# wujinzhong/seamlessCloneOptimization

Hardware: AMD Instinct MI355X
Metric: Mpix/s seamlessClone (ROI 2048^2) (higher is better)
Workload: dtype f32 (arithmetic); storage: 16-bit fixed-point field on the first two level-0 stores of a solve, float16 right-hand side and level 1

## Files before the change

include/seamlessclone_hip_testing.h:

```cpp
#ifndef SEAMLESSCLONE_HIP_TESTING_H
#define SEAMLESSCLONE_HIP_TESTING_H

#include "seamlessclone_hip.h"

#ifdef __cplusplus
extern "C" {
#endif

#define SC_FLAG_LEGACY_PATHS   (1 << 6)
#define SC_LEGACY_SEPARATE_RESTRICT 1
#define SC_LEGACY_BOTTOM_F32   2
#define SC_LEGACY_SEPARATE_TAIL 4
#define SC_LEGACY_UNPACKED_TILES 8
#define SC_FLAG_KEEP_FIELD     (1 << 7)

#define SC_FLAG_POISON_ARENA   (1 << 14)


SC_API int sc_hip_mask_stage(void *instance, const uint8_t *mask, int mask_cols, int mask_rows, int mask_step,
                      int centerX, int centerY, int geo[6], uint8_t *M_out, size_t M_capacity);

SC_API int sc_hip_build_rhs(void *instance,
                     const uint8_t *face, int face_cols, int face_rows, int face_step,
                     const uint8_t *body, int body_cols, int body_rows, int body_step,
                     const uint8_t *mask, int mask_cols, int mask_rows, int mask_step,
                     int centerX, int centerY, int geo[6], float *B_out, float *lap_out, size_t plane_capacity);

SC_API int sc_hip_edit_rhs(void *instance, const sc_edit_params *p, const uint8_t *src, int cols, int rows, int src_step,
// ... 12 lines not shown
SC_API int sc_hip_field_finish(void *instance, uint8_t *body, int body_cols, int body_rows, int body_step, int ltx, int lty);
SC_API int sc_hip_field_lowmode(void *instance);

SC_API int sc_hip_field_time_sweeps(void *instance, int method, int launches, int sweeps_per_launch, float omega,
                             float *ms_per_launch);

SC_API int sc_hip_time_cycle0(void *instance, int launches, float *ms_per_launch);
SC_API int sc_hip_time_cycle0_form(void *instance, int form, int launches, float *ms_per_launch);
SC_API int sc_hip_time_coarse_chain(void *instance, int reps, float *ms_eager, float *ms_graph, int *launches);
SC_API int sc_hip_time_tail_phases(void *instance, unsigned long long *cycles11);

SC_API int sc_hip_selftest_host(void);

SC_API int sc_hip_cycle0_form(const int *facts, int index, int form[3]);

SC_API int sc_hip_coarse_tile_plan(const int *facts, int *plan);

#define SC_FUSED_ROW 18
SC_API int sc_hip_fused_schedule(const int *facts, const int *verdicts, int nverdicts, int *rows, int capacity);

SC_API int sc_hip_restore_spans(long long step, int rows, int ltx, int lty, int W, int H, long long *spans, int capacity);

#ifdef __cplusplus
}
#endif
#endif
```

seamlesscloneoptimization_amd/capi.py:

```python
from __future__ import annotations

import ctypes as C
import os
import re
import subprocess

import numpy as np

_PKG = os.path.dirname(os.path.abspath(__file__))
_ROOT = os.path.dirname(_PKG)
LIB_PATH = os.path.join(_PKG, "libseamlessclone_hip.so")
HEADER_PATH = os.path.join(_ROOT, "include", "seamlessclone_hip.h")
TESTING_HEADER_PATH = os.path.join(_ROOT, "include", "seamlessclone_hip_testing.h")

SC_OK = 0
SC_ERR_BAD_ARG = -1
SC_ERR_BAD_SIZE = -2
SC_ERR_EMPTY_MASK = -3
SC_ERR_ROI_OOB = -4
SC_ERR_HIP = -5
SC_ERR_NOT_CONVERGED = -6

SC_NORMAL_CLONE = 1
SC_MIXED_CLONE = 2
# ... 14 lines not shown
SC_METHOD_FFT = 6
SC_AUTO_DIRECT_MAX = 720
SC_AUTO_DIRECT_AREA = 450000
SC_AUTO_NARROW_MAX = 140
SC_AUTO_THIN_MAX = 4
SC_AUTO_THIN_LONG_MAX = 4096

SC_FLAG_NO_SPECULATE = 1 << 0
SC_FLAG_FLOAT_RHS = 1 << 1
SC_FLAG_FLOAT_U0 = 1 << 2
SC_FLAG_NO_COMPOSE_L1 = 1 << 3
SC_FLAG_VCYCLE_BOTTOM = 1 << 4
SC_FLAG_EXACT_TABLES = 1 << 5
SC_FLAG_LEGACY_PATHS = 1 << 6
SC_LEGACY_SEPARATE_RESTRICT, SC_LEGACY_BOTTOM_F32, SC_LEGACY_SEPARATE_TAIL, SC_LEGACY_UNPACKED_TILES = 1, 2, 4, 8
SC_FLAG_KEEP_FIELD = 1 << 7
SC_FLAG_FFT_FP64 = 1 << 8
SC_FLAG_OPENCV_GREY_MASK = 1 << 9
SC_FLAG_FLOAT_L1 = 1 << 10
SC_FLAG_FLOAT_FIELD = 1 << 11
SC_FLAG_NO_STAGE_MARKS = 1 << 12
SC_FLAG_ROWS_RETURN = 1 << 13
SC_FLAG_POISON_ARENA = 1 << 14

def auto_takes_direct(w: int, h: int) -> bool:
    if w <= SC_AUTO_DIRECT_MAX and h <= SC_AUTO_DIRECT_MAX:
        return True
    if max(w, h) <= SC_AUTO_THIN_LONG_MAX and (w * h <= SC_AUTO_DIRECT_AREA or min(w, h) <= SC_AUTO_NARROW_MAX):
        return True
    return False
# ... 234 lines not shown
    L.sc_hip_device_count.restype = C.c_int
    L.sc_hip_device_pci_bus_id.argtypes = [C.c_int, C.c_char_p, C.c_int]
    L.sc_hip_device_pci_bus_id.restype = C.c_int
    L.sc_hip_mask_stage.argtypes = [C.c_void_p] + _IMG + [C.c_int, C.c_int, i32p, u8p, C.c_size_t]
    L.sc_hip_mask_stage.restype = C.c_int
    L.sc_hip_build_rhs.argtypes = [C.c_void_p] + _IMG * 3 + [C.c_int, C.c_int, i32p, f32p, f32p, C.c_size_t]
    L.sc_hip_build_rhs.restype = C.c_int
    L.sc_hip_field_load.argtypes = [C.c_void_p, C.c_int, C.c_int, C.c_int, f32p, f32p]
    L.sc_hip_field_load.restype = C.c_int
    L.sc_hip_field_sweep.argtypes = [C.c_void_p, C.c_int, C.c_int, C.c_float, C.c_int]
    L.sc_hip_field_sweep.restype = C.c_int
    L.sc_hip_field_residual.argtypes = [C.c_void_p, f64p]
    L.sc_hip_field_residual.restype = C.c_int
    L.sc_hip_field_solve.argtypes = [C.c_void_p]
    L.sc_hip_field_solve.restype = C.c_int
    L.sc_hip_field_shape.argtypes = [C.c_void_p, i32p]
    L.sc_hip_field_shape.restype = C.c_int
    L.sc_hip_field_store.argtypes = [C.c_void_p, f32p, C.c_size_t]
    L.sc_hip_field_store.restype = C.c_int
    L.sc_hip_field_finish.argtypes = [C.c_void_p, C.c_void_p, C.c_int, C.c_int, C.c_int, C.c_int, C.c_int]
    L.sc_hip_field_finish.restype = C.c_int
    L.sc_hip_field_lowmode.argtypes = [C.c_void_p]
    L.sc_hip_field_lowmode.restype = C.c_int
    L.sc_hip_field_time_sweeps.argtypes = [C.c_void_p, C.c_int, C.c_int, C.c_int, C.c_float, C.POINTER(C.c_float)]
    L.sc_hip_field_time_sweeps.restype = C.c_int
    L.sc_hip_pool_create.argtypes = [C.c_int, C.c_int]
    L.sc_hip_pool_create.restype = C.c_void_p
    L.sc_hip_pool_destroy.argtypes = [C.c_void_p]
    L.sc_hip_pool_destroy.restype = None
    L.sc_hip_pool_size.argtypes = [C.c_void_p]
# ... 588 lines not shown
        cap = m[1] * m[2]
        B = np.zeros(3 * cap, np.float32)
        lap = np.zeros(3 * cap, np.float32)
        self._check(self.L.sc_hip_build_rhs(self.h, *f, *b, *m, int(cx), int(cy), geo.ctypes.data_as(i32p),
                                            B.ctypes.data_as(f32p), lap.ctypes.data_as(f32p), cap))
        W, H = int(geo[2]), int(geo[3])
        return geo, B[:3 * W * H].reshape(3, H, W).copy(), lap[:3 * W * H].reshape(3, H, W).copy()

    def field_load(self, U, lap):
        U = np.ascontiguousarray(U, np.float32)
        lap = np.ascontiguousarray(lap, np.float32)
        assert U.shape == lap.shape and U.ndim == 3
        Cc, H, W = U.shape
        self._check(self.L.sc_hip_field_load(self.h, W, H, Cc, U.ctypes.data_as(f32p), lap.ctypes.data_as(f32p)))

    def field_shape(self):
        whc = np.zeros(3, np.int32)
        self._check(self.L.sc_hip_field_shape(self.h, whc.ctypes.data_as(i32p)))
        return int(whc[2]), int(whc[1]), int(whc[0])

    def field_sweep(self, method, sweeps, omega=1.0, sweeps_per_launch=1):
        self._check(self.L.sc_hip_field_sweep(self.h, int(method), int(sweeps), float(omega), int(sweeps_per_launch)))

    def field_residual(self):
        out = np.zeros(2, np.float64)
        self._check(self.L.sc_hip_field_residual(self.h, out.ctypes.data_as(f64p)))
        return float(out[0]), float(out[1])

    def field_solve(self, allow_not_converged=False):
        rc = self.L.sc_hip_field_solve(self.h)
# ... 167 lines not shown

def plan_prepare(sizes, opts: "SolverOpts | None" = None) -> int:
    wh = np.ascontiguousarray(np.asarray(sizes, np.int32).reshape(-1, 2))
    return int(load().sc_hip_plan_prepare(wh.ctypes.data_as(i32p), wh.shape[0], C.byref(opts) if opts is not None else None))


def plan_cache_clear() -> None:
    load().sc_hip_plan_cache_clear()


CYCLE0_FACTS = ("sweeps", "prolong", "f_half", "u_half", "q16_in", "q16_out", "final_cycle", "out_bytes", "composed", "l1_half", "timing",
                "bands", "rag")


def cycle0_form(**facts):
    f = (C.c_int * len(CYCLE0_FACTS))(*[int(facts.pop(k, 0)) for k in CYCLE0_FACTS])
    if facts:
        raise TypeError("cycle0_form: no such fact: %s" % sorted(facts))
    out = (C.c_int * 3)()
    return tuple(out) if load().sc_hip_cycle0_form(f, 0, out) == 0 else -1


def coarse_tile_plan(W, H, C_, useful, halo, rows, size_class=False, unpacked=False, lanes=False):
    f = (C.c_int * 10)(W, H, C_, useful, halo, rows, int(size_class), int(unpacked), 0, 0)
    head = np.zeros(4, np.int32)
    rc = load().sc_hip_coarse_tile_plan(f, head.ctypes.data_as(i32p))
    if rc != 0:
        raise SeamlessCloneError(rc, "coarse_tile_plan")
    if not lanes:
        return tuple(int(v) for v in head)
# ... 80 lines not shown
```

seamlesscloneoptimization_amd/csrc/sc_common.h:

```cpp
#pragma once
#include <hip/hip_runtime.h>
#include <stdint.h>
#include <stddef.h>
#include <algorithm>
#include <string>
#include <vector>
#include "../../include/seamlessclone_hip_testing.h"

namespace sc {

struct Field {
    float *p = nullptr;
    int W = 0, H = 0, C = 0;
    int pitch = 0;
    size_t plane = 0;
    __host__ __device__ float *at(int c) const { return p + (size_t)c * plane; }
    size_t bytes() const { return plane * (size_t)C * sizeof(float); }
};

static inline int round_up(int v, int m) { return (v + m - 1) / m * m; }

struct Geo { int x0, y0, W, H, ltx, lty; };

struct Img8 {
// ... 198 lines not shown
struct MGGeom { MGDim x, y; };
struct ComposeArgs { Field E2; MGGeom g1; };

constexpr int C0_TIMING   = 1;
constexpr int C0_F_HALF   = 2;
constexpr int C0_U_HALF   = 4;
constexpr int C0_FINAL    = 8;
constexpr int C0_COMPOSED = 16;
constexpr int C0_OUT      = 32;
constexpr int C0_BANDS    = 64;
constexpr int C0_L1_HALF  = 128;
constexpr int C0_Q16_IN   = 256;
constexpr int C0_Q16_OUT  = 512;
constexpr int C0_PACK_ROWS = 6;
constexpr int C0_PACK     = 2048;
constexpr int C0_RAG      = 1024;

struct Cycle0Launch {
    Field Uin, Uout, F, Fc, E;
    MGGeom g{};
    int sweeps = 0;
    bool prolong = false;
    bool f_half = false, u_half = false, q16_in = false, q16_out = false;
    bool final_cycle = false, out_bytes = false;
    bool composed = false;
    bool l1_half = false, timing = false;
    ComposeArgs comp{};
    float4 *bands = nullptr;
    float *partial = nullptr;
    LmNodes lm{};
    AbortFlag sat{};
    const RagMember *rag = nullptr;
    hipStream_t s = nullptr;
};
bool cycle0_form(const Cycle0Launch &d, int &T, bool &PRO, int &TAG);
int  cycle0_form_at(int i, int &T, bool &PRO, int &TAG);
int  launch_cycle0(const Cycle0Launch &d);

constexpr int RAG_MAX_LEVELS = 12;
// ... 44 lines not shown
```

seamlesscloneoptimization_amd/csrc/sc_cycle0.hip:

```cpp
#include "sc_common.h"
#include <hip/hip_fp16.h>
#include "sc_wave.h"
#include "sc_mg_device.h"
#include <type_traits>

namespace sc {

constexpr int C0_HXQ = 3;
constexpr int C0_HX = 4 * C0_HXQ;

template <int R>
__device__ __forceinline__ void c0_load(const float *__restrict__ p, int P, int H, int x, int y0, float4 (&v)[R])
{
    const int xc = min(max(x, 0), P - 4);
#pragma unroll
    for (int r = 0; r < R; ++r) {
        const int yc = min(max(y0 + r, 0), H - 1);
        v[r] = *reinterpret_cast<const float4 *>(p + (size_t)yc * P + xc);
    }
}

template <int R>
__device__ __forceinline__ void c0_load_half(const __half *__restrict__ p, int P, int H, int x, int y0, float4 (&v)[R])
{
// ... 64 lines not shown
    else asm("v_fma_mix_f32 %0, %1, %2, %3 op_sel_hi:[0,0,1]" : "=v"(d) : "v"(s), "s"(quarter), "v"(raw));
    return d;
}
template <int K>
__device__ __forceinline__ float c0_f_minus(const uint2 &h, float s)
{
    const unsigned raw = (K < 2) ? h.x : h.y;
    float d;
    if (K & 1) asm("v_fma_mix_f32 %0, %1, -4.0, -%2 op_sel:[1,0,0] op_sel_hi:[1,0,0]" : "=v"(d) : "v"(raw), "v"(s));
    else asm("v_fma_mix_f32 %0, %1, -4.0, -%2 op_sel_hi:[1,0,0]" : "=v"(d) : "v"(raw), "v"(s));
    return d;
}
__device__ __forceinline__ float c0_comp(const float4 &v, int k) { return k == 0 ? v.x : k == 1 ? v.y : k == 2 ? v.z : v.w; }


template <int T, int NW, int R, bool PRO, bool GEN, bool ZEROIN, int TAG = 0>
__global__ __launch_bounds__(NW * 64) __attribute__((amdgpu_waves_per_eu(4))) void k_cycle0(Field Uin, Field Uout, Field F, Field Fc, Field E, MGGeom g,
                                                    float *__restrict__ partial, ComposeArgs comp, float4 *__restrict__ bands, LmNodes lm, AbortFlag sat,
                                                    const RagMember *__restrict__ rag, int lev)
{
    constexpr int HY = 2 * T + 2, RH = NW * R;
    constexpr bool RAG = (TAG & C0_RAG) != 0;
    constexpr bool COMP = (TAG & C0_COMPOSED) != 0;
    static_assert(!COMP || (PRO && !GEN && R % 2 == 0), "composition of two prolongations exists on level 0 only");
    constexpr bool FINAL = (TAG & C0_FINAL) != 0;
    constexpr bool OUT = (TAG & C0_OUT) != 0, BANDS = ((TAG & C0_BANDS) != 0 || FINAL) && !OUT;
    static_assert(!OUT || (FINAL && !GEN), "bytes leave from the last level-0 launch only");
    static_assert(!(TAG & C0_BANDS) || !GEN, "cell shares exist on level 0 only");
    constexpr bool HF = (TAG & C0_F_HALF) != 0, HU = (TAG & C0_U_HALF) != 0;
    static_assert(!(HF && GEN), "float16 right-hand sides exist on level 0 only");
    constexpr bool L1H = (TAG & C0_L1_HALF) != 0;
    constexpr bool UQI = (TAG & C0_Q16_IN) != 0, UQO = (TAG & C0_Q16_OUT) != 0;
    static_assert(!((UQI || UQO) && (GEN || (HU && UQI) || (OUT && UQO))), "16-bit fields: level 0, between its launches");
    static_assert(!L1H || !GEN || ZEROIN, "float16 level-1 fields: the level-1 launch starts from a zero correction");
    static_assert(!(PRO && GEN), "the in-kernel prolongation relies on level 0's regular last interval");
    static_assert(2 * T + 2 <= C0_HX, "column halo too small");
    static_assert(R % 2 == 0, "bands must hold whole coarse-row pairs");
    __shared__ float4 edge[2][NW][2][64];
    __shared__ float2 hedge[2][NW][64];
    const int lane = threadIdx.x & 63;
    const int wv = __builtin_amdgcn_readfirstlane(threadIdx.x >> 6);
    int W = Uin.W, H = Uin.H;
    const int P = Uin.pitch;
    const int nbx = (W + (256 - 2 * C0_HX) - 1) / (256 - 2 * C0_HX), nby = (H + (RH - 2 * HY) - 1) / (RH - 2 * HY);
    const int tile = xcd_tile(blockIdx.x, gridDim.x);
    constexpr bool PACK = (TAG & C0_PACK) != 0;
    static_assert(!PACK || (GEN && ZEROIN && !PRO && !RAG), "packed column tiles: the coarse forms of one size");
    TileLane tl{};
    if constexpr (PACK) tl = coarse_tile_lane(coarse_tile_plan(W, H, Uin.C, 256 - 2 * C0_HX, C0_HX, RH - 2 * HY, false), Uin.C, 256 - 2 * C0_HX, C0_HX, tile, lane);
    const int bx = tile % nbx, by = PACK ? tl.by : (tile / nbx) % nby;
    const int c = PACK ? min(tl.c, Uin.C - 1) : tile / (nbx * nby);
    const int sl = PACK ? tl.sl : lane, lps = PACK ? tl.lps : 64;
    const bool live = !PACK || tl.c < Uin.C;
    if constexpr (RAG) {
        const RagMember &m = rag[c / 3];
        W = m.lw[lev]; H = m.lh[lev];
        if (bx * (256 - 2 * C0_HX) >= W || by * (RH - 2 * HY) >= H) {
            if (PRO && threadIdx.x == 0) partial[tile] = 0.f;
            return;
        }
        g = m.g[lev];
        if (PRO) E.H = m.lh[lev + 1];
        if ((TAG & C0_COMPOSED) != 0) { comp.g1 = m.g[lev + 1]; comp.E2.H = m.lh[lev + 2]; }
    }
    const int x = PACK ? tl.x : bx * (256 - 2 * C0_HX) - C0_HX + 4 * lane;
    const int y0 = by * (RH - 2 * HY) - HY + wv * R;
    float4 u[R], f[HF ? 1 : R];
    uint2 fh[HF ? R : 1];
    if (ZEROIN) {
#pragma unroll
        for (int r = 0; r < R; ++r) u[r] = make_float4(0.f, 0.f, 0.f, 0.f);
    } else if (HU) {
        c0_load_half<R>(reinterpret_cast<const __half *>(Uin.p) + (size_t)c * Uin.plane, P, H, x, y0, u);
    } else if (UQI) {
        c0_load_q16<R>(reinterpret_cast<const uint16_t *>(Uin.p) + (size_t)c * Uin.plane, P, H, x, y0, u);
    } else {
        c0_load<R>(Uin.at(c), P, H, x, y0, u);
    }
    constexpr int NE = R / 2 + 2, NQ = R / 4 + 3;
    float2 eab[PRO ? NE : 1];
    float ecc[PRO ? NE : 1];
// ... 135 lines not shown
                    m2 = fmaxf(fmaxf(m2, fabsf(Sj.y)), fabsf(Sj.w));
                }
                Sp = Sj;
            }
            m = fmaxf(m1, fmaxf(0.5f * m2, 0.25f * m4));
        };
        if (inner) prolong(std::false_type{});
        else if (x >= 0 && x <= W - 2 && y0 + R - 1 >= 1 && y0 <= H - 2) prolong(std::true_type{});
        if constexpr (HF) c0_load_half_raw<R>(reinterpret_cast<const __half *>(F.p) + (size_t)c * F.plane, P, H, x, y0, fh);
        else c0_load<R>(F.at(c), P, H, x, y0, f);
#pragma unroll
        for (int o = 32; o > 0; o >>= 1) m = fmaxf(m, __shfl_xor(m, o, 64));
        __shared__ float red[NW];
        if (lane == 0) red[wv] = m;
        __syncthreads();
        if (threadIdx.x == 0) {
            float mm = red[0];
#pragma unroll
            for (int w = 1; w < NW; ++w) mm = fmaxf(mm, red[w]);
            partial[tile] = mm;
        }
    }

    if constexpr (!GEN) {
#pragma unroll
        for (int r = 0; r < R; ++r) {
            if constexpr (HF) c0_scale_q(fh[r]);
            else f[r] = make_float4(-0.25f * f[r].x, -0.25f * f[r].y, -0.25f * f[r].z, -0.25f * f[r].w);
        }
    }
    const float quarter = 0.25f;
    (void)quarter;
    float cw0 = (GEN && x + 0 == g.x.n) ? g.x.cw_last : 1.0f, dx0 = (GEN && x + 0 == g.x.n) ? g.x.d_last : 2.0f;
    float cw1 = (GEN && x + 1 == g.x.n) ? g.x.cw_last : 1.0f, dx1 = (GEN && x + 1 == g.x.n) ? g.x.d_last : 2.0f;
    float cw2 = (GEN && x + 2 == g.x.n) ? g.x.cw_last : 1.0f, dx2 = (GEN && x + 2 == g.x.n) ? g.x.d_last : 2.0f;
// ... 167 lines not shown
                v1 = __builtin_fmaf(h1[r + 1], 0.5f, __builtin_fmaf(m1, 0.5f, h1[r]));
            }
            const float fy = (J == g.y.nc) ? 2.0f * g.y.inv_last : 1.0f;
            if constexpr (L1H && !GEN) {
                __half *o = reinterpret_cast<__half *>(Fc.p) + (size_t)c * Fc.plane + (size_t)J * Fc.pitch + I;
                if (I >= 1 && I <= g.x.nc) o[0] = __float2half_rn(v0 * (fx0 * fy));
                if (I + 1 >= 1 && I + 1 <= g.x.nc) o[1] = __float2half_rn(v1 * (fx1 * fy));
            } else {
            float *o = fc + (size_t)J * Fc.pitch + I;
            if (I >= 1 && I <= g.x.nc) o[0] = v0 * (fx0 * fy);
            if (I + 1 >= 1 && I + 1 <= g.x.nc) o[1] = v1 * (fx1 * fy);
            }
        }
    }

    if (sl < C0_HXQ || sl >= lps - C0_HXQ || !live || x >= P || x >= W) return;
    if constexpr (OUT) {
        uint8_t *__restrict__ q = reinterpret_cast<uint8_t *>(Uout.p) + (size_t)c * Uout.plane;
        const bool corr = lm.CN && x <= W - 2;
        const int Yc0 = max(y0, 0) >> 3;
        float nd[3][2] = { { 0.f, 0.f }, { 0.f, 0.f }, { 0.f, 0.f } };
        if (corr) {
            const float *__restrict__ pn = lm.CN + (size_t)c * lm.ny * lm.npitch + (x >> 3);
#pragma unroll
            for (int k = 0; k < 3; ++k) {
                const float *row = pn + (size_t)min(Yc0 + k, lm.ny - 1) * lm.npitch;
                nd[k][0] = row[0]; nd[k][1] = row[1];
            }
        }
#pragma unroll
        for (int r = 0; r < R; ++r) {
            const int yr = wv * R + r, y = y0 + r;
            if (!(yr >= HY && yr < RH - HY && y >= 1 && y <= H - 2)) continue;
            float4 v = u[r];
            if (corr) {
                const bool second = (y >> 3) != Yc0;
                lm_add4_nodes(second ? nd[1][0] : nd[0][0], second ? nd[1][1] : nd[0][1], second ? nd[2][0] : nd[1][0], second ? nd[2][1] : nd[1][1], x, y, v);
            }
            *reinterpret_cast<unsigned *>(q + (size_t)y * P + x) = lm_byte(v.x) | (lm_byte(v.y) << 8) | (lm_byte(v.z) << 16) | (lm_byte(v.w) << 24);
        }
        return;
    }
    if constexpr (GEN && L1H) {
        __half *__restrict__ outh = reinterpret_cast<__half *>(Uout.p) + (size_t)c * Uout.plane;
#pragma unroll
        for (int r = 0; r < R; ++r) {
            const int yr = wv * R + r, y = y0 + r;
            if (!(yr >= HY && yr < RH - HY && y >= 0 && y < H)) continue;
            const __half2 a = __floats2half2_rn(u[r].x, u[r].y), b2 = __floats2half2_rn(u[r].z, u[r].w);
            uint2 pk; pk.x = *reinterpret_cast<const unsigned *>(&a); pk.y = *reinterpret_cast<const unsigned *>(&b2);
            *reinterpret_cast<uint2 *>(outh + (size_t)y * P + x) = pk;
        }
        return;
    }
    if constexpr (UQO) {
        uint16_t *__restrict__ outq = reinterpret_cast<uint16_t *>(Uout.p) + (size_t)c * Uout.plane;
// ... 4 lines not shown
            if (!(yr >= HY && yr < RH - HY && y >= 0 && y < H)) continue;
            uint2 pk;
            pk.x = c0_q16_checked(u[r].x, s0) | (c0_q16_checked(u[r].y, s1) << 16);
            pk.y = c0_q16_checked(u[r].z, s2) | (c0_q16_checked(u[r].w, s3) << 16);
            *reinterpret_cast<uint2 *>(outq + (size_t)y * P + x) = pk;
        }
        const int seen = s0 | (x + 1 < W ? s1 : 0) | (x + 2 < W ? s2 : 0) | (x + 3 < W ? s3 : 0);
        if ((seen & ~0xffff) && sat.p) { *sat.p = sat.gen; if (sat.host) *sat.host = sat.gen; }
        return;
    }
    float *__restrict__ out = Uout.at(c);
#pragma unroll
    for (int r = 0; r < R; ++r) {
        const int yr = wv * R + r, y = y0 + r;
        if (yr >= HY && yr < RH - HY && y >= 0 && y < H) *reinterpret_cast<float4 *>(out + (size_t)y * P + x) = u[r];
    }
}

constexpr int C0_NW = 8, C0_R = 8;


using Cycle0Kernel = void (*)(Field, Field, Field, Field, Field, MGGeom, float *, ComposeArgs, float4 *, LmNodes, AbortFlag, const RagMember *, int);
struct Cycle0Form { int T; bool PRO; int TAG; Cycle0Kernel k; };
#define C0_FORM(T_, PRO_, TAG_) { T_, PRO_, TAG_, k_cycle0<T_, C0_NW, C0_R, PRO_, false, false, TAG_> }
#define C0_FORM_RAG(T_, PRO_, TAG_) C0_FORM(T_, PRO_, TAG_), C0_FORM(T_, PRO_, TAG_ | C0_RAG)
#define C0_FORM_TWIN(T_, PRO_, TAG_) C0_FORM(T_, PRO_, TAG_), C0_FORM(T_, PRO_, TAG_ | C0_TIMING)
constexpr int C0_FAST = C0_F_HALF | C0_L1_HALF, C0_FAST_CYCLE = C0_FAST | C0_COMPOSED, C0_Q16 = C0_Q16_IN | C0_Q16_OUT;
static constexpr Cycle0Form c0_forms[] = {
    C0_FORM_RAG(2, false, C0_FAST | C0_U_HALF | C0_Q16_OUT), C0_FORM(2, false, C0_FAST | C0_U_HALF | C0_Q16_OUT | C0_TIMING),
    C0_FORM_RAG(2, false, C0_FAST | C0_U_HALF), C0_FORM_RAG(2, false, C0_FAST),
// ... 6 lines not shown
    C0_FORM_TWIN(4, true, C0_COMPOSED | C0_F_HALF), C0_FORM(4, true, C0_COMPOSED | C0_F_HALF | C0_BANDS),
    C0_FORM(2, true, C0_COMPOSED | C0_F_HALF | C0_FINAL), C0_FORM(2, true, C0_COMPOSED | C0_F_HALF | C0_FINAL | C0_OUT),
    C0_FORM_TWIN(4, true, C0_COMPOSED), C0_FORM(4, true, C0_COMPOSED | C0_BANDS),
    C0_FORM(2, true, C0_COMPOSED | C0_FINAL), C0_FORM(2, true, C0_COMPOSED | C0_FINAL | C0_OUT),
    C0_FORM(1, false, C0_F_HALF | C0_U_HALF), C0_FORM(2, false, C0_F_HALF | C0_U_HALF),
    C0_FORM_TWIN(1, false, C0_F_HALF), C0_FORM_TWIN(2, false, C0_F_HALF), C0_FORM_TWIN(1, false, 0), C0_FORM_TWIN(2, false, 0),
    C0_FORM_TWIN(2, true, C0_F_HALF), C0_FORM_TWIN(3, true, C0_F_HALF), C0_FORM_TWIN(4, true, C0_F_HALF), C0_FORM(4, true, C0_F_HALF | C0_BANDS),
    C0_FORM_TWIN(2, true, 0), C0_FORM_TWIN(3, true, 0), C0_FORM_TWIN(4, true, 0), C0_FORM(4, true, C0_BANDS),
    C0_FORM(1, true, C0_F_HALF | C0_FINAL), C0_FORM(2, true, C0_F_HALF | C0_FINAL), C0_FORM(2, true, C0_F_HALF | C0_FINAL | C0_OUT),
    C0_FORM(1, true, C0_FINAL), C0_FORM(2, true, C0_FINAL), C0_FORM(2, true, C0_FINAL | C0_OUT),
};
#undef C0_FORM_TWIN
#undef C0_FORM_RAG
#undef C0_FORM

static const Cycle0Form *c0_find(const Cycle0Launch &d)
{
    const bool shares = d.bands && d.prolong && !d.final_cycle && d.sweeps == 4;
    const int TAG = (d.timing ? C0_TIMING : 0) | (d.f_half ? C0_F_HALF : 0) | (d.u_half ? C0_U_HALF : 0) | (d.final_cycle ? C0_FINAL : 0) |
                    (d.composed ? C0_COMPOSED : 0) | (d.out_bytes ? C0_OUT : 0) | (shares ? C0_BANDS : 0) | (d.l1_half ? C0_L1_HALF : 0) |
                    (d.q16_in ? C0_Q16_IN : 0) | (d.q16_out ? C0_Q16_OUT : 0) | (d.rag ? C0_RAG : 0);
    for (const Cycle0Form &f : c0_forms)
        if (f.TAG == TAG && f.T == d.sweeps && f.PRO == d.prolong) return &f;
    return nullptr;
}

bool cycle0_form(const Cycle0Launch &d, int &T, bool &PRO, int &TAG)
{
    const Cycle0Form *f = c0_find(d);
    if (f) { T = f->T; PRO = f->PRO; TAG = f->TAG; }
    return f != nullptr;
}
int cycle0_form_at(int i, int &T, bool &PRO, int &TAG)
{
    const int n = (int)(sizeof(c0_forms) / sizeof(c0_forms[0]));
    if (i >= 0 && i < n) { T = c0_forms[i].T; PRO = c0_forms[i].PRO; TAG = c0_forms[i].TAG; }
    return n;
}

int launch_cycle0(const Cycle0Launch &d)
{
    const Cycle0Form *f = c0_find(d);
    if (!f) return -1;
    const int blocks = cycle0_blocks(d.Uin.W, d.Uin.H, d.Uin.C, f->T);
    hipLaunchKernelGGL(f->k, dim3(blocks), dim3(C0_NW * 64), 0, d.s, d.Uin, d.Uout, d.F, d.Fc, d.E, d.g, d.partial, d.comp, d.bands, d.lm, d.sat, d.rag, 0);
    return f->PRO ? blocks : 0;
}

void cycle0_row_geometry(int H, int sweeps, int &nby, int &step, int &hy)
{
    const int RH = C0_NW * C0_R;
    hy = 2 * sweeps + 2; step = RH - 2 * hy; nby = (H + step - 1) / step;
}

int cycle0_blocks(int W, int H, int C, int sweeps)
{
// ... 56 lines not shown
```

seamlesscloneoptimization_amd/csrc/sc_hooks.cpp:

```cpp
#include "sc_instance.h"
#include <algorithm>
#include <cmath>
#include <cstring>
#include <vector>

using namespace sc;

static int float_rhs(Instance *I)
{
    if (!I->f_half) return SC_OK;
    SC_HIP(I, hipSetDevice(I->gpu));
    Field scratch = I->result_in_U1 ? I->U0 : I->U1;
    const size_t n = I->F.plane * (size_t)I->F.C;
    launch_half_to_float(I->F.p, scratch.p, n, I->stream);
    SC_HIP(I, hipGetLastError());
    SC_HIP(I, hipMemcpyAsync(I->F.p, scratch.p, n * sizeof(float), hipMemcpyDeviceToDevice, I->stream));
    I->f_half = false;
    return SC_OK;
}

static int mg_time_coarse_chain(Instance *I, int reps, float *ms_eager, float *ms_graph, int *launches)
{
    if (I->mg.size() < 4 || I->mg_bottom < 3 || !mg_composes_level1(I)) { I->err = "time_coarse_chain: run a multigrid clone of at least ~500^2 first"; return SC_ERR_BAD_ARG; }
    const int pre = mg_params(I->opts).pre, post = mg_params(I->opts).post;
// ... 220 lines not shown
        for (size_t i = 0; i < (size_t)cols * rows; ++i) edges_out[i] = edges_out[i] == 2 ? 255 : 0;
    }
    if (counts) { counts[0] = I->hyst_launches; counts[1] = I->hyst_reads; }
    SC_HIP(I, hipStreamSynchronize(I->stream));
    return SC_OK;
}

int sc_hip_edit_counts(void *p, int counts[2])
{
    Instance *I = get(p);
    if (!I || !counts) return SC_ERR_BAD_ARG;
    counts[0] = I->hyst_launches; counts[1] = I->hyst_reads;
    return SC_OK;
}

int sc_hip_field_load(void *p, int W, int H, int C, const float *U, const float *lap)
{
    Instance *I = get(p);
    if (I) field_moved(I);
    if (I) I->out_direct = false;
    if (!I || !U || !lap) return SC_ERR_BAD_ARG;
    I->err.clear();
    SC_HIP(I, hipSetDevice(I->gpu));
    if (W < 1 || H < 1 || C < 1 || C > 16) return SC_ERR_BAD_SIZE;
    int rc;
    if ((rc = setup_fields(I, W, H, C))) return rc;
    SC_HIP(I, hipMemsetAsync(I->d_U0.p, 0, I->U0.bytes(), I->stream));
    SC_HIP(I, hipMemsetAsync(I->d_U1.p, 0, I->U1.bytes(), I->stream));
    SC_HIP(I, hipMemsetAsync(I->d_F.p, 0, I->F.bytes(), I->stream));
    const size_t wb = (size_t)W * sizeof(float), pb = (size_t)I->U0.pitch * sizeof(float);
// ... 200 lines not shown
        }
    }
    return SC_OK;
}

int sc_hip_cycle0_form(const int *facts, int index, int form[3])
{
    if (!form) return SC_ERR_BAD_ARG;
    int T = 0, TAG = 0, rc;
    bool PRO = false;
    if (facts) {
        static float4 some_bands;
        static const RagMember some_class{};
        Cycle0Launch d;
        d.sweeps = facts[0]; d.prolong = facts[1]; d.f_half = facts[2]; d.u_half = facts[3]; d.q16_in = facts[4]; d.q16_out = facts[5];
        d.final_cycle = facts[6]; d.out_bytes = facts[7]; d.composed = facts[8]; d.l1_half = facts[9]; d.timing = facts[10];
        d.bands = facts[11] ? &some_bands : nullptr; d.rag = facts[12] ? &some_class : nullptr;
        rc = cycle0_form(d, T, PRO, TAG) ? 0 : -1;
    } else if ((rc = cycle0_form_at(index, T, PRO, TAG)) <= index || index < 0) {
        return rc;
    }
    if (rc >= 0) { form[0] = T; form[1] = PRO; form[2] = TAG; }
    return rc;
}

int sc_hip_fused_schedule(const int *facts, const int *verdicts, int nverdicts, int *rows, int capacity)
{
    if (!facts || !rows || nverdicts < 0 || (nverdicts > 0 && !verdicts)) return SC_ERR_BAD_ARG;
    const int pre = facts[0], post = facts[1], budget = facts[2], early_kind = facts[9];
    if (pre < 1 || pre > 2 || post < 1 || post > 2 || budget < 1 || budget > 64 || early_kind < 0 || early_kind > 3) return SC_ERR_BAD_ARG;
    const bool bytes_form = facts[10] != 0;
// ... 41 lines not shown
```

seamlesscloneoptimization_amd/csrc/sc_instance.h:

```cpp
#pragma once
#include "sc_common.h"
#include "sc_hostcopy.h"
#include <algorithm>
#include <memory>
#include <cmath>

namespace sc {

struct DevBuf {
    void *p = nullptr;
    size_t cap = 0;
    bool own = true;
};
inline void dev_release(DevBuf &b) { if (b.p && b.own) (void)hipFree(b.p); b.p = nullptr; b.cap = 0; }

struct FD1 {
    int n = 0;
    float cw_last = 0.f, d_last = 0.f;
    std::vector<double> lam, q, ee;
};

struct LowMode {
    int w = 0, h = 0, C = 0;
    int Kx = 0, Ky = 0, Kxp = 0, Kyp = 0;
// ... 106 lines not shown
    DevBuf d_face, d_body_roi, d_mask, d_out;
    DevBuf h_face, h_body, h_mask, h_out;
    DevBuf h_sx, h_sy;
    std::unique_ptr<RowCopier> copier;
    hipEvent_t ev_chunk[8]{};
    DevBuf d_M;
    int mpitch = 0;
    DevBuf d_edge, h_hyst;
    int hyst_launches = 0, hyst_reads = 0;
    DevBuf d_pois;
    bool auto_as_single = false;
    float screen_lambda = 0.f;
    DevBuf d_U0, d_U1, d_F;
    Field U0, U1, F;
    bool result_in_U1 = false;
    bool out_direct = false;
    bool f_half = false;
    bool u_half = false;
    bool u_q16 = false;
    bool mg_q16_last = false;
    AbortFlag sat;
    unsigned sat_counter = 0;
    bool force_float_field = false;
    struct SpecPost { SolveTarget to; bool armed = false, done = false; } spec_post;
    RectGuard guard;
    int last_mc = -1, last_mr = -1, last_rect[4] = { 0, 0, 0, 0 };
    int spec_cooldown = 0;
    bool erode_done = false;
    BboxTask pending_scan;
    bool scan_pending = false;
// ... 45 lines not shown
};

struct CallScope {
    Instance *I;
    ~CallScope()
    {
        I->edit_call = false;
        I->force_float_field = false;
        I->spec_post = Instance::SpecPost();
        I->auto_as_single = false;
        I->screen_lambda = 0.f;
    }
};

inline bool legacy_path(const sc_solver_opts &o, int which) { return (o.flags & SC_FLAG_LEGACY_PATHS) && (o.legacy_paths & which); }

constexpr int SC_RETRY_FLOAT_FIELD = 1;

int hip_fail(Instance *I, hipError_t e, const char *what);
#define SC_HIP(I, call)                                                   \
    do {                                                                  \
        hipError_t e_ = (call);                                           \
        if (e_ != hipSuccess) return hip_fail((I), e_, #call);            \
    } while (0)

int ensure(Instance *I, DevBuf &b, size_t bytes, bool zero = true);
int ensure_pinned(Instance *I, DevBuf &b, size_t bytes);
double fd_selftest_error();
double fd_closed_selftest_error();
int setup_fields(Instance *I, int W, int H, int C);
// ... 214 lines not shown
```

seamlesscloneoptimization_amd/csrc/sc_multigrid.cpp:

```cpp
#include "sc_instance.h"
#include <algorithm>
#include <cmath>
#include <cstring>
#include <cstdlib>

namespace sc {

static int run_bottom(Instance *I, size_t l0, int pre, int post)
{
    MGBottomArgs a;
    a.nlevels = (int)(I->mg.size() - l0);
    a.pre = pre; a.post = post;
    const MGLevel &last = I->mg.back();
    a.coarse_sweeps = std::max(8, std::min(64, 2 * std::max(last.g.x.n, last.g.y.n)));
    int off = 0;
    for (int i = 0; i < a.nlevels; ++i) {
        const MGLevel &L = I->mg[l0 + i];
        a.lv[i].g = L.g; a.lv[i].omega = L.omega;
        a.lv[i].pitch = bottom_pitch(L);
        const int plane = a.lv[i].pitch * (L.g.y.n + 2);
        a.lv[i].offU = off; a.lv[i].offF = off + plane;
        off += 2 * plane;
    }
    a.fd_level = I->fd_level; a.fd_nxp = I->fd_nxp; a.fd_nyp = I->fd_nyp;
// ... 332 lines not shown
        if (s.kind == FUSED_DONE) break;
        verdict = VERDICT_NONE;
        if (s.coarse_first && (rc = vcycle(I, 1, pre, post, s.composed ? (1u << 1) : 0u))) return rc;
        if (s.ask_early) fused_early(S, s, lowmode_early_kind(I, utol));
        if (s.coarse_first) bands = s.bands_sweeps ? lowmode_bands_buffer(I, s.bands_sweeps) : nullptr;
        if (s.lm && I->aux_pending) {
            SC_HIP(I, hipStreamWaitEvent(I->stream, I->ev_join, 0));
            I->aux_pending = false;
        }
        float *const part_now = part_base + (size_t)((S.cyc + 1) & 1) * nb_cap;
        Cycle0Launch d = step_launch(level0_launch(I, s.composed), s);
        if (s.prolong) d.partial = part_now;
        if (s.bands) d.bands = bands;
        if (s.lm) d.lm = early_lm;
        if (s.sat) d.sat = sat;
        const int nb = launch_cycle0(d);
        if (s.out_bytes && nb <= 0) { verdict = VERDICT_NO_FORM; continue; }
        if (s.prolong ? nb <= 0 : nb < 0) { I->err = "cycle0: unsupported depth"; return SC_ERR_BAD_ARG; }
        const Field Q = I->result_in_U1 ? I->U0 : I->U1;
        if (!s.out_bytes) I->result_in_U1 = !I->result_in_U1;
        if (s.kind == FUSED_FIRST) {
            if (I->rag.dev && I->rag.ready_pending) {
                SC_HIP(I, hipStreamWaitEvent(I->stream, I->rag.ev_ready, 0));
                I->rag.ready_pending = false;
            }
            I->u_half = false;
            I->mg_q16_last = q16;
        } else if (!s.out_bytes) {
            lowmode_bands_written(I, d.bands ? result(I).p : nullptr);
        }
        I->u_q16 = s.q16_out;
        if (s.nodes != NODES_NONE) {
            early_lm = LmNodes();
            if (s.nodes == NODES_MAIN) {
// ... 4 lines not shown
                if ((rc = lowmode_nodes(I, result(I), early_lm, I->aux))) return rc;
                SC_HIP(I, hipEventRecord(I->ev_join, I->aux));
                I->aux_pending = true;
            }
        }
        if (!s.prolong) continue;
        SC_HIP(I, hipGetLastError());
        const int nb_prev = nb_last;
        if (!s.out_bytes) nb_last = nb;
        if (!s.judged) continue;
        float m, m_prev;
        bool saturated = false;
        if (s.out_bytes)
            rc = correction_maxima(I, maxima, S.cyc + 1, nb, nb_prev, part_now, [&]() -> int {
                    const SolveTarget &to = I->spec_post.to;
                    if (!to.group) launch_splice_planar(Q, to.org, to.step, I->stream, I->guard, sat);
                    else launch_splice_planar_group(Q, to.group->data(), (int)to.group->size(), I->stream, sat);
                    return SC_OK;
                }, m, m_prev, saturated);
        else
            rc = correction_maxima(I, maxima, S.cyc + 1, nb, nb_prev, part_now, [&]() -> int {
                    if (!(I->spec_post.armed && o.tol <= 0.f)) return SC_OK;
                    const int lrc = write_output(I, I->spec_post.to, sat);
                    if (lrc) return lrc;
                    I->spec_post.done = true;
                    return SC_OK;
                }, m, m_prev, saturated);
        if (rc) return rc;
        I->info.last_update = m;
        bool stop = false;
// ... 68 lines not shown
```

Before: 23030.

## Fuse interleaved RGB byte output into final level-0 cycle kernel

In the final judged bytes-output cycle, each workgroup now processes all three channels of a tile in a loop, stages the per-channel bytes in shared memory, then writes interleaved 3-channel pixels directly into the body image. This removes the separate planar splice launch and the planar byte intermediate round trip for same-size groups with enough tiles. The cost is a third as many blocks, each doing three times the work serially, plus extra LDS use that may reduce occupancy.

```diff
diff --git a/include/seamlessclone_hip_testing.h b/include/seamlessclone_hip_testing.h
--- a/include/seamlessclone_hip_testing.h
+++ b/include/seamlessclone_hip_testing.h
@@ -12,6 +12,8 @@
 #define SC_LEGACY_BOTTOM_F32   2
 #define SC_LEGACY_SEPARATE_TAIL 4
 #define SC_LEGACY_UNPACKED_TILES 8
+#define SC_LEGACY_SPLICE_LAUNCH 16
+#define SC_FORCE_INTERLEAVED_OUT 32
 #define SC_FLAG_KEEP_FIELD     (1 << 7)
 
 #define SC_FLAG_POISON_ARENA   (1 << 14)
@@ -54,6 +56,8 @@
 
 SC_API int sc_hip_cycle0_form(const int *facts, int index, int form[3]);
 
+SC_API int sc_hip_bytes_writer(void *instance);
+
 SC_API int sc_hip_coarse_tile_plan(const int *facts, int *plan);
 
 #define SC_FUSED_ROW 18
diff --git a/seamlesscloneoptimization_amd/capi.py b/seamlesscloneoptimization_amd/capi.py
--- a/seamlesscloneoptimization_amd/capi.py
+++ b/seamlesscloneoptimization_amd/capi.py
@@ -52,6 +52,8 @@
 SC_FLAG_EXACT_TABLES = 1 << 5
 SC_FLAG_LEGACY_PATHS = 1 << 6
 SC_LEGACY_SEPARATE_RESTRICT, SC_LEGACY_BOTTOM_F32, SC_LEGACY_SEPARATE_TAIL, SC_LEGACY_UNPACKED_TILES = 1, 2, 4, 8
+SC_LEGACY_SPLICE_LAUNCH = 16
+SC_FORCE_INTERLEAVED_OUT = 32
 SC_FLAG_KEEP_FIELD = 1 << 7
 SC_FLAG_FFT_FP64 = 1 << 8
 SC_FLAG_OPENCV_GREY_MASK = 1 << 9
@@ -316,6 +318,8 @@
     L.sc_hip_field_residual.restype = C.c_int
     L.sc_hip_field_solve.argtypes = [C.c_void_p]
     L.sc_hip_field_solve.restype = C.c_int
+    L.sc_hip_bytes_writer.argtypes = [C.c_void_p]
+    L.sc_hip_bytes_writer.restype = C.c_int
     L.sc_hip_field_shape.argtypes = [C.c_void_p, i32p]
     L.sc_hip_field_shape.restype = C.c_int
     L.sc_hip_field_store.argtypes = [C.c_void_p, f32p, C.c_size_t]
@@ -934,6 +938,9 @@
         Cc, H, W = U.shape
         self._check(self.L.sc_hip_field_load(self.h, W, H, Cc, U.ctypes.data_as(f32p), lap.ctypes.data_as(f32p)))
 
+    def bytes_writer(self):
+        return int(self.L.sc_hip_bytes_writer(self.h))
+
     def field_shape(self):
         whc = np.zeros(3, np.int32)
         self._check(self.L.sc_hip_field_shape(self.h, whc.ctypes.data_as(i32p)))
@@ -1131,6 +1138,8 @@
 
 
 def cycle0_form(**facts):
+    if facts.pop("out_interleaved", 0):
+        facts["out_bytes"] = int(bool(facts.get("out_bytes", 0))) | 2
     f = (C.c_int * len(CYCLE0_FACTS))(*[int(facts.pop(k, 0)) for k in CYCLE0_FACTS])
     if facts:
         raise TypeError("cycle0_form: no such fact: %s" % sorted(facts))
diff --git a/seamlesscloneoptimization_amd/csrc/sc_common.h b/seamlesscloneoptimization_amd/csrc/sc_common.h
--- a/seamlesscloneoptimization_amd/csrc/sc_common.h
+++ b/seamlesscloneoptimization_amd/csrc/sc_common.h
@@ -236,6 +236,7 @@
 constexpr int C0_Q16_OUT  = 512;
 constexpr int C0_PACK_ROWS = 6;
 constexpr int C0_PACK     = 2048;
+constexpr int C0_OUT3     = 4096;
 constexpr int C0_RAG      = 1024;
 
 struct Cycle0Launch {
@@ -245,6 +246,8 @@
     bool prolong = false;
     bool f_half = false, u_half = false, q16_in = false, q16_out = false;
     bool final_cycle = false, out_bytes = false;
+    bool out_interleaved = false;
+    const ImageJob *jobs = nullptr; int njobs = 0;
     bool composed = false;
     bool l1_half = false, timing = false;
     ComposeArgs comp{};
diff --git a/seamlesscloneoptimization_amd/csrc/sc_cycle0.hip b/seamlesscloneoptimization_amd/csrc/sc_cycle0.hip
--- a/seamlesscloneoptimization_amd/csrc/sc_cycle0.hip
+++ b/seamlesscloneoptimization_amd/csrc/sc_cycle0.hip
@@ -102,18 +102,63 @@
 __device__ __forceinline__ float c0_comp(const float4 &v, int k) { return k == 0 ? v.x : k == 1 ? v.y : k == 2 ? v.z : v.w; }
 
 
-template <int T, int NW, int R, bool PRO, bool GEN, bool ZEROIN, int TAG = 0>
+constexpr int C0_OUT3_ROWS = 52, C0_OUT3_WORDS = (256 - 2 * C0_HX) / 4;
+__device__ __forceinline__ int c0_lane_again() { int z = 0; asm volatile("" : "+v"(z)); return (int)__builtin_amdgcn_mbcnt_hi(~0u, __builtin_amdgcn_mbcnt_lo(~0u, (unsigned)z)); }
+template <bool ON> __device__ __forceinline__ float c0_opaque_s(float v) { if constexpr (ON) asm volatile("" : "+s"(v)); return v; }
+template <bool ON> __device__ __forceinline__ int c0_opaque_s(int v) { if constexpr (ON) asm volatile("" : "+s"(v)); return v; }
+template <int N> __device__ __forceinline__ unsigned *c0_out3_stage() { __shared__ unsigned stage[N]; return stage; }
+__device__ __forceinline__ void c0_out3_write(const unsigned *__restrict__ stage, uint8_t *__restrict__ body, int bstep, int W, int H, int x0t, int y0t,
+                                              int wv, int lane, int nw)
+{
+    const int lo = 3 * (max(x0t, 1) - x0t), hi = 3 * (min(x0t + 4 * C0_OUT3_WORDS, W - 1) - x0t);
+    for (int rr = wv; rr < C0_OUT3_ROWS; rr += nw) {
+        const int y = y0t + rr;
+        if (y < 1 || y > H - 2) continue;
+        uint8_t *d = body + (size_t)y * bstep + 3 * (size_t)x0t;
+        const int a = (int)((uintptr_t)d & 3);
+        const int o0 = 12 * lane - a;
+        if (o0 >= hi || o0 + 12 <= lo) continue;
+        const int jc = min(lane, C0_OUT3_WORDS - 1), jp = max(min(lane - 1, C0_OUT3_WORDS - 1), 0);
+        unsigned pc[3], pp[3];
+#pragma unroll
+        for (int c = 0; c < 3; ++c) {
+            const unsigned *row = stage + (c * C0_OUT3_ROWS + rr) * C0_OUT3_WORDS;
+            pc[c] = row[jc]; pp[c] = row[jp];
+        }
+        unsigned w[4];
+        w[0] = ((pp[2] >> 16) & 255u) | ((pp[0] >> 24) << 8) | ((pp[1] >> 24) << 16) | ((pp[2] >> 24) << 24);
+        w[1] = (pc[0] & 255u) | ((pc[1] & 255u) << 8) | ((pc[2] & 255u) << 16) | (((pc[0] >> 8) & 255u) << 24);
+        w[2] = ((pc[1] >> 8) & 255u) | (((pc[2] >> 8) & 255u) << 8) | (((pc[0] >> 16) & 255u) << 16) | (((pc[1] >> 16) & 255u) << 24);
+        w[3] = ((pc[2] >> 16) & 255u) | ((pc[0] >> 24) << 8) | ((pc[1] >> 24) << 16) | ((pc[2] >> 24) << 24);
+#pragma unroll
+        for (int k = 0; k < 3; ++k) {
+            const unsigned v = (unsigned)(((((unsigned long long)w[k + 1]) << 32) | w[k]) >> (8 * (4 - a)));
+            const int o = o0 + 4 * k;
+            if (o >= lo && o + 4 <= hi) *reinterpret_cast<unsigned *>(d + o) = v;
+            else {
+#pragma unroll
+                for (int b = 0; b < 4; ++b)
+                    if (o + b >= lo && o + b < hi) d[o + b] = (uint8_t)(v >> (8 * b));
+            }
+        }
+    }
+}
+
+template <int T, int NW, int R, bool PRO, bool GEN, bool ZEROIN, int TAG = 0, class... X3>
 __global__ __launch_bounds__(NW * 64) __attribute__((amdgpu_waves_per_eu(4))) void k_cycle0(Field Uin, Field Uout, Field F, Field Fc, Field E, MGGeom g,
                                                     float *__restrict__ partial, ComposeArgs comp, float4 *__restrict__ bands, LmNodes lm, AbortFlag sat,
-                                                    const RagMember *__restrict__ rag, int lev)
+                                                    const RagMember *__restrict__ rag, int lev, X3... x3)
 {
     constexpr int HY = 2 * T + 2, RH = NW * R;
+    constexpr bool OUT3 = (TAG & C0_OUT3) != 0;
+    static_assert(sizeof...(X3) == (OUT3 ? 1 : 0), "the members' jobs travel with the three-channel bytes form only");
     constexpr bool RAG = (TAG & C0_RAG) != 0;
     constexpr bool COMP = (TAG & C0_COMPOSED) != 0;
     static_assert(!COMP || (PRO && !GEN && R % 2 == 0), "composition of two prolongations exists on level 0 only");
     constexpr bool FINAL = (TAG & C0_FINAL) != 0;
     constexpr bool OUT = (TAG & C0_OUT) != 0, BANDS = ((TAG & C0_BANDS) != 0 || FINAL) && !OUT;
     static_assert(!OUT || (FINAL && !GEN), "bytes leave from the last level-0 launch only");
+    static_assert(!OUT3 || (OUT && !RAG && T == 2 && RH - 2 * HY == C0_OUT3_ROWS), "interleaved bytes: the judged two-sweep form of a same-size group");
     static_assert(!(TAG & C0_BANDS) || !GEN, "cell shares exist on level 0 only");
     constexpr bool HF = (TAG & C0_F_HALF) != 0, HU = (TAG & C0_U_HALF) != 0;
     static_assert(!(HF && GEN), "float16 right-hand sides exist on level 0 only");
@@ -137,11 +182,11 @@
     TileLane tl{};
     if constexpr (PACK) tl = coarse_tile_lane(coarse_tile_plan(W, H, Uin.C, 256 - 2 * C0_HX, C0_HX, RH - 2 * HY, false), Uin.C, 256 - 2 * C0_HX, C0_HX, tile, lane);
     const int bx = tile % nbx, by = PACK ? tl.by : (tile / nbx) % nby;
-    const int c = PACK ? min(tl.c, Uin.C - 1) : tile / (nbx * nby);
+    const int c_first = PACK ? min(tl.c, Uin.C - 1) : OUT3 ? 3 * (tile / (nbx * nby)) : tile / (nbx * nby);
     const int sl = PACK ? tl.sl : lane, lps = PACK ? tl.lps : 64;
     const bool live = !PACK || tl.c < Uin.C;
     if constexpr (RAG) {
-        const RagMember &m = rag[c / 3];
+        const RagMember &m = rag[c_first / 3];
         W = m.lw[lev]; H = m.lh[lev];
         if (bx * (256 - 2 * C0_HX) >= W || by * (RH - 2 * HY) >= H) {
             if (PRO && threadIdx.x == 0) partial[tile] = 0.f;
@@ -151,8 +196,22 @@
         if (PRO) E.H = m.lh[lev + 1];
         if ((TAG & C0_COMPOSED) != 0) { comp.g1 = m.g[lev + 1]; comp.E2.H = m.lh[lev + 2]; }
     }
+    const int lane_wg = lane, wv_wg = wv, bx_wg = bx, by_wg = by;
+    const MGGeom &g_wg = g;
+    const ComposeArgs &comp_wg = comp;
+    int ci = 0, c_run = c_first, pt_run = OUT3 ? tile + 2 * (c_first / 3) * (nbx * nby) : tile;
+    const int pt_step = nbx * nby;
+    _Pragma("nounroll") do {
+    const int lane = OUT3 ? c0_lane_again() : lane_wg, wv = c0_opaque_s<OUT3>(wv_wg), bx = c0_opaque_s<OUT3>(bx_wg), by = c0_opaque_s<OUT3>(by_wg);
+    std::conditional_t<OUT3, MGGeom, const MGGeom &> g = g_wg;
+    std::conditional_t<OUT3, ComposeArgs, const ComposeArgs &> comp = comp_wg;
+    if constexpr (OUT3) {
+        g.x.tw1 = c0_opaque_s<OUT3>(g.x.tw1); g.y.tw1 = c0_opaque_s<OUT3>(g.y.tw1);
+        comp.g1.x.tw1 = c0_opaque_s<OUT3>(comp.g1.x.tw1); comp.g1.y.tw1 = c0_opaque_s<OUT3>(comp.g1.y.tw1);
+    }
     const int x = PACK ? tl.x : bx * (256 - 2 * C0_HX) - C0_HX + 4 * lane;
     const int y0 = by * (RH - 2 * HY) - HY + wv * R;
+    const int c = OUT3 ? c_run : c_first, ptile = OUT3 ? pt_run : tile;
     float4 u[R], f[HF ? 1 : R];
     uint2 fh[HF ? R : 1];
     if (ZEROIN) {
@@ -318,11 +377,11 @@
         __shared__ float red[NW];
         if (lane == 0) red[wv] = m;
         __syncthreads();
-        if (threadIdx.x == 0) {
+        if (OUT3 ? (lane == 0 && wv == 0) : threadIdx.x == 0) {
             float mm = red[0];
 #pragma unroll
             for (int w = 1; w < NW; ++w) mm = fmaxf(mm, red[w]);
-            partial[tile] = mm;
+            partial[ptile] = mm;
         }
     }
 
@@ -520,7 +579,9 @@
         }
     }
 
-    if (sl < C0_HXQ || sl >= lps - C0_HXQ || !live || x >= P || x >= W) return;
+    if constexpr (OUT3) {
+        if (lane < C0_HXQ || lane >= 64 - C0_HXQ || x >= P || x >= W) continue;
+    } else if (sl < C0_HXQ || sl >= lps - C0_HXQ || !live || x >= P || x >= W) return;
     if constexpr (OUT) {
         uint8_t *__restrict__ q = reinterpret_cast<uint8_t *>(Uout.p) + (size_t)c * Uout.plane;
         const bool corr = lm.CN && x <= W - 2;
@@ -543,9 +604,11 @@
                 const bool second = (y >> 3) != Yc0;
                 lm_add4_nodes(second ? nd[1][0] : nd[0][0], second ? nd[1][1] : nd[0][1], second ? nd[2][0] : nd[1][0], second ? nd[2][1] : nd[1][1], x, y, v);
             }
-            *reinterpret_cast<unsigned *>(q + (size_t)y * P + x) = lm_byte(v.x) | (lm_byte(v.y) << 8) | (lm_byte(v.z) << 16) | (lm_byte(v.w) << 24);
-        }
-        return;
+            const unsigned px4 = lm_byte(v.x) | (lm_byte(v.y) << 8) | (lm_byte(v.z) << 16) | (lm_byte(v.w) << 24);
+            if constexpr (OUT3) c0_out3_stage<3 * C0_OUT3_ROWS * C0_OUT3_WORDS>()[(ci * C0_OUT3_ROWS + (yr - HY)) * C0_OUT3_WORDS + (lane - C0_HXQ)] = px4;
+            else *reinterpret_cast<unsigned *>(q + (size_t)y * P + x) = px4;
+        }
+        if constexpr (OUT3) continue; else return;
     }
     if constexpr (GEN && L1H) {
         __half *__restrict__ outh = reinterpret_cast<__half *>(Uout.p) + (size_t)c * Uout.plane;
@@ -580,6 +643,15 @@
     for (int r = 0; r < R; ++r) {
         const int yr = wv * R + r, y = y0 + r;
         if (yr >= HY && yr < RH - HY && y >= 0 && y < H) *reinterpret_cast<float4 *>(out + (size_t)y * P + x) = u[r];
+    }
+    } while (OUT3 && (c_run += 1, pt_run += pt_step, ++ci < 3));
+    if constexpr (OUT3) {
+        const ImageJobs &t = (x3, ...);
+        const ImageJob &j = t.j[c_first / 3];
+        __syncthreads();
+        if (abort_set(sat)) return;
+        if (j.d_rect && (j.d_rect[0] != j.rx0 || j.d_rect[1] != j.rx1 || j.d_rect[2] != j.ry0 || j.d_rect[3] != j.ry1)) return;
+        c0_out3_write(c0_out3_stage<3 * C0_OUT3_ROWS * C0_OUT3_WORDS>(), j.body_org, j.bstep, W, H, bx * (256 - 2 * C0_HX), by * (RH - 2 * HY), wv, c0_lane_again(), NW);
     }
 }
 
@@ -616,8 +688,16 @@
 #undef C0_FORM_RAG
 #undef C0_FORM
 
+constexpr int C0_OUT3_TAG = C0_FAST_CYCLE | C0_FINAL | C0_OUT | C0_OUT3;
+static bool c0_is_out3(const Cycle0Launch &d)
+{
+    return d.out_interleaved && d.out_bytes && d.final_cycle && d.prolong && d.composed && d.sweeps == 2 && d.f_half && d.l1_half && !d.u_half && !d.q16_in &&
+           !d.q16_out && !d.timing && !d.rag;
+}
+
 static const Cycle0Form *c0_find(const Cycle0Launch &d)
 {
+    if (d.out_interleaved) return nullptr;
     const bool shares = d.bands && d.prolong && !d.final_cycle && d.sweeps == 4;
     const int TAG = (d.timing ? C0_TIMING : 0) | (d.f_half ? C0_F_HALF : 0) | (d.u_half ? C0_U_HALF : 0) | (d.final_cycle ? C0_FINAL : 0) |
                     (d.composed ? C0_COMPOSED : 0) | (d.out_bytes ? C0_OUT : 0) | (shares ? C0_BANDS : 0) | (d.l1_half ? C0_L1_HALF : 0) |
@@ -629,6 +709,7 @@
 
 bool cycle0_form(const Cycle0Launch &d, int &T, bool &PRO, int &TAG)
 {
+    if (c0_is_out3(d)) { T = 2; PRO = true; TAG = C0_OUT3_TAG; return true; }
     const Cycle0Form *f = c0_find(d);
     if (f) { T = f->T; PRO = f->PRO; TAG = f->TAG; }
     return f != nullptr;
@@ -642,6 +723,15 @@
 
 int launch_cycle0(const Cycle0Launch &d)
 {
+    if (d.out_interleaved) {
+        if (!c0_is_out3(d) || !d.jobs || d.njobs < 1 || d.njobs > (int)ImageJobs::MAX || d.Uin.C != 3 * d.njobs) return -1;
+        ImageJobs t{};
+        for (int i = 0; i < d.njobs; ++i) t.j[i] = d.jobs[i];
+        const int blocks = cycle0_blocks(d.Uin.W, d.Uin.H, d.njobs, 2);
+        hipLaunchKernelGGL((k_cycle0<2, C0_NW, C0_R, true, false, false, C0_OUT3_TAG, ImageJobs>), dim3(blocks), dim3(C0_NW * 64), 0, d.s, d.Uin, d.Uout, d.F, d.Fc,
+                           d.E, d.g, d.partial, d.comp, d.bands, d.lm, d.sat, d.rag, 0, t);
+        return 3 * blocks;
+    }
     const Cycle0Form *f = c0_find(d);
     if (!f) return -1;
     const int blocks = cycle0_blocks(d.Uin.W, d.Uin.H, d.Uin.C, f->T);
diff --git a/seamlesscloneoptimization_amd/csrc/sc_hooks.cpp b/seamlesscloneoptimization_amd/csrc/sc_hooks.cpp
--- a/seamlesscloneoptimization_amd/csrc/sc_hooks.cpp
+++ b/seamlesscloneoptimization_amd/csrc/sc_hooks.cpp
@@ -258,6 +258,15 @@
     return SC_OK;
 }
 
+int sc_hip_bytes_writer(void *p)
+{
+    Instance *I = get(p);
+    if (!I) return SC_ERR_BAD_ARG;
+    const int w = I->bytes_writer;
+    I->bytes_writer = 0;
+    return w;
+}
+
 int sc_hip_field_load(void *p, int W, int H, int C, const float *U, const float *lap)
 {
     Instance *I = get(p);
@@ -488,7 +497,7 @@
         static const RagMember some_class{};
         Cycle0Launch d;
         d.sweeps = facts[0]; d.prolong = facts[1]; d.f_half = facts[2]; d.u_half = facts[3]; d.q16_in = facts[4]; d.q16_out = facts[5];
-        d.final_cycle = facts[6]; d.out_bytes = facts[7]; d.composed = facts[8]; d.l1_half = facts[9]; d.timing = facts[10];
+        d.final_cycle = facts[6]; d.out_bytes = (facts[7] & 1) != 0; d.out_interleaved = (facts[7] & 2) != 0; d.composed = facts[8]; d.l1_half = facts[9]; d.timing = facts[10];
         d.bands = facts[11] ? &some_bands : nullptr; d.rag = facts[12] ? &some_class : nullptr;
         rc = cycle0_form(d, T, PRO, TAG) ? 0 : -1;
     } else if ((rc = cycle0_form_at(index, T, PRO, TAG)) <= index || index < 0) {
diff --git a/seamlesscloneoptimization_amd/csrc/sc_instance.h b/seamlesscloneoptimization_amd/csrc/sc_instance.h
--- a/seamlesscloneoptimization_amd/csrc/sc_instance.h
+++ b/seamlesscloneoptimization_amd/csrc/sc_instance.h
@@ -144,6 +144,7 @@
     DevBuf d_U0, d_U1, d_F;
     Field U0, U1, F;
     bool result_in_U1 = false;
+    int bytes_writer = 0;
     bool out_direct = false;
     bool f_half = false;
     bool u_half = false;
@@ -219,6 +220,7 @@
 };
 
 inline bool legacy_path(const sc_solver_opts &o, int which) { return (o.flags & SC_FLAG_LEGACY_PATHS) && (o.legacy_paths & which); }
+constexpr long SC_OUT3_MIN_TILES = 200;
 
 constexpr int SC_RETRY_FLOAT_FIELD = 1;
 
diff --git a/seamlesscloneoptimization_amd/csrc/sc_multigrid.cpp b/seamlesscloneoptimization_amd/csrc/sc_multigrid.cpp
--- a/seamlesscloneoptimization_amd/csrc/sc_multigrid.cpp
+++ b/seamlesscloneoptimization_amd/csrc/sc_multigrid.cpp
@@ -370,10 +370,24 @@
         if (s.bands) d.bands = bands;
         if (s.lm) d.lm = early_lm;
         if (s.sat) d.sat = sat;
+        bool interleaved = false;
+        if (s.out_bytes) {
+            const SolveTarget &to = I->spec_post.to;
+            if (to.group && !d.rag && to.group->size() <= (size_t)ImageJobs::MAX && to.group->size() * 3 == (size_t)I->F.C && (*to.group)[0].W == 0 &&
+                !legacy_path(o, SC_LEGACY_SPLICE_LAUNCH)) {
+                const long tiles = (long)cycle0_blocks(I->F.W, I->F.H, (int)to.group->size(), s.sweeps);
+                Cycle0Launch d3 = d;
+                d3.out_interleaved = true; d3.jobs = to.group->data(); d3.njobs = (int)to.group->size(); d3.sat = sat;
+                int T3, TAG3;
+                bool PRO3;
+                if ((tiles >= SC_OUT3_MIN_TILES || legacy_path(o, SC_FORCE_INTERLEAVED_OUT)) && cycle0_form(d3, T3, PRO3, TAG3)) { d = d3; interleaved = true; }
+            }
+        }
         const int nb = launch_cycle0(d);
         if (s.out_bytes && nb <= 0) { verdict = VERDICT_NO_FORM; continue; }
         if (s.prolong ? nb <= 0 : nb < 0) { I->err = "cycle0: unsupported depth"; return SC_ERR_BAD_ARG; }
         const Field Q = I->result_in_U1 ? I->U0 : I->U1;
+        if (s.out_bytes) I->bytes_writer |= interleaved ? 2 : 1;
         if (!s.out_bytes) I->result_in_U1 = !I->result_in_U1;
         if (s.kind == FUSED_FIRST) {
             if (I->rag.dev && I->rag.ready_pending) {
@@ -408,6 +422,7 @@
         if (s.out_bytes)
             rc = correction_maxima(I, maxima, S.cyc + 1, nb, nb_prev, part_now, [&]() -> int {
                     const SolveTarget &to = I->spec_post.to;
+                    if (interleaved) return SC_OK;
                     if (!to.group) launch_splice_planar(Q, to.org, to.step, I->stream, I->guard, sat);
                     else launch_splice_planar_group(Q, to.group->data(), (int)to.group->size(), I->stream, sat);
                     return SC_OK;
```

Measured after the change: 23740, median of 6. 3.1% higher.
